# jianwen-xie/Latent-Space-Normalizing-Flow

Hardware: AMD Instinct MI355X
Metric: latent-samples/sec through flow+logdet, nz=128 B=65536 (higher is better)
Workload: dtype bf16x3; 1 GPU; CIFAR-10 flow prior nz=128 f_width=64 f_depth=5 affine, forward+logdet+log-prob, B=65536 synthetic z per evaluation (BASELINE.json configs[2]); rows_per_gpu=65536, global_rows=65536, parallelism=single GPU, streams=3, clock_ramp_launches_before_warmup=600

## Files before the change

### latent-space-normalizing-flow_amd/csrc/lsnf_device.h

```cpp
#pragma once
#include <hip/hip_runtime.h>
#include <type_traits>
#include "lsnf_layout.h"

typedef float f32x16 __attribute__((ext_vector_type(16)));
typedef float f32x4 __attribute__((ext_vector_type(4)));

#define LSNF_WG_THREADS 256
#define LSNF_WG_WAVES 4
#define LSNF_WG_SAMPLES (LSNF_WG_WAVES * 32)

#define LSNF_AS1 __attribute__((address_space(1)))
#define LSNF_AS3 __attribute__((address_space(3)))

static inline hipError_t lsnf_allow_big_lds(const void* kernel, unsigned long long* done_mask) {
    int dev = 0;
    hipError_t e = hipGetDevice(&dev);
    if (e != hipSuccess) return e;
    if (dev >= 0 && dev < 64 && ((*done_mask >> dev) & 1ull)) return hipSuccess;
    e = hipFuncSetAttribute(kernel, hipFuncAttributeMaxDynamicSharedMemorySize, 160 * 1024);
    if (e != hipSuccess) return e;
    if (dev >= 0 && dev < 64) *done_mask |= 1ull << dev;
    return hipSuccess;
}
// ... 7 lines not shown

static inline unsigned long long* lsnf_stamps_buffer() {
#ifdef LSNF_STAMPS
    extern unsigned long long* g_lsnf_stamps;
    if (!g_lsnf_stamps && hipMalloc(&g_lsnf_stamps, sizeof(unsigned long long) * 64 * 4 * 4096) != hipSuccess) g_lsnf_stamps = nullptr;
    return g_lsnf_stamps;
#else
    return nullptr;
#endif
}

template <int HT_, int WT_>
struct LsnfStackCfg {
    static constexpr int HT = HT_, WT = WT_, NZT = 2 * HT_;
    static constexpr int P1 = NZT, P2 = WT, P3 = WT, P4 = 2 * HT, NP = P1 + P2 + P3 + P4;
    static constexpr int KT1 = NZT, KT2 = HT, KT3 = WT, KT4 = WT;
    static constexpr int OFF_S2 = LSNF_FRAG_FLOATS * P1 * KT1;
    static constexpr int OFF_S3 = OFF_S2 + LSNF_FRAG_FLOATS * P2 * KT2;
    static constexpr int OFF_S4 = OFF_S3 + LSNF_FRAG_FLOATS * P3 * KT3;
    static constexpr int FWD_BLOCK = OFF_S4 + LSNF_FRAG_FLOATS * P4 * KT4;
    static constexpr int FWD_CONST = 32 * NP + 32;
    static constexpr int INV_BLOCK = LSNF_FRAG_FLOATS * NZT * NZT;
    static constexpr int INV_CONST = 32 * NZT;
    static constexpr int OFF_B4 = 0;
    static constexpr int OFF_B3 = OFF_B4 + LSNF_FRAG_FLOATS * WT * 2 * HT;
    static constexpr int OFF_B2 = OFF_B3 + LSNF_FRAG_FLOATS * WT * WT;
    static constexpr int OFF_B1 = OFF_B2 + LSNF_FRAG_FLOATS * HT * WT;
    static constexpr int BWD_BLOCK = OFF_B1 + LSNF_FRAG_FLOATS * NZT * NZT;
    static constexpr int MAXKT = (NZT > WT ? NZT : WT);
    static constexpr int SLOT = 2 * MAXKT * LSNF_FRAG_FLOATS;
};

#define LSNF_STATS_SLOTS 64
__device__ __forceinline__ void lsnf_publish_stats(double* stats, double sum_ll, double sum_logdet, int rows, int lane) {
    const unsigned grid = gridDim.x, wg = blockIdx.x;
    unsigned long long* ticket = reinterpret_cast<unsigned long long*>(&stats[2]);
    int last = 0;
    if (lane == 0) {
        const unsigned s = wg % LSNF_STATS_SLOTS;
        double* sub = stats + 8 + 4 * s;
        const double r0 = atomicAdd(&sub[0], sum_ll);
        const double r1 = atomicAdd(&sub[1], sum_logdet);
        unsigned long long inc = 1ull;
        asm volatile("" : "+v"(inc) : "v"(r0), "v"(r1));
        bool slot_done = true;
        if (grid > LSNF_STATS_SLOTS) {
            const unsigned long long n_s = (grid - s + LSNF_STATS_SLOTS - 1) / LSNF_STATS_SLOTS;
            unsigned long long* st = reinterpret_cast<unsigned long long*>(&sub[2]);
            slot_done = atomicAdd(st, inc) == n_s - 1;
            if (slot_done) atomicExch(st, 0ull);
            inc = 1ull;
        }
        if (slot_done) {
            const unsigned long long slots = grid > LSNF_STATS_SLOTS ? LSNF_STATS_SLOTS : grid;
            if (atomicAdd(ticket, inc) == slots - 1) { last = 1; atomicExch(ticket, 0ull); }
        }
    }
    if (__builtin_amdgcn_readfirstlane(last)) {
        unsigned long long* sub = reinterpret_cast<unsigned long long*>(stats + 8 + 4 * lane);
        double fl = __longlong_as_double((long long)atomicExch(&sub[0], 0ull));
        double fd = __longlong_as_double((long long)atomicExch(&sub[1], 0ull));
#pragma unroll
        for (int o = 32; o > 0; o >>= 1) { fl += __shfl_xor(fl, o, 64); fd += __shfl_xor(fd, o, 64); }
        if (lane == 0) { stats[4] = fl; stats[5] = fd; stats[6] = (double)rows; }
    }
}

__device__ __forceinline__ constexpr int lsnf_feat(int r, int h) { return (r & 3) + 8 * (r >> 2) + 4 * h; }

template <int KT, int NW = LSNF_WG_WAVES>
__device__ __forceinline__ void lsnf_issue_panel(const float* __restrict__ gsrc, float* lbuf, int wave, int lane) {
#ifdef LSNF_ABLATE_DMA
    return;
#endif
    constexpr int PIECES = 4 * KT;
    constexpr int PER_WAVE = (PIECES + NW - 1) / NW;
#pragma unroll
    for (int s = 0; s < PER_WAVE; ++s) {
        const int seg = s * NW + wave;
        if (PIECES % NW == 0 || seg < PIECES) {
            const float* g = gsrc + seg * 256 + lane * 4;
            float* l = lbuf + seg * 256;
            __builtin_amdgcn_global_load_lds((const LSNF_AS1 void*)g, (LSNF_AS3 void*)l, 16, 0, 0);
        }
    }
}

__device__ __forceinline__ void lsnf_panel_barrier() {
    asm volatile("s_waitcnt vmcnt(0)" ::: "memory");
#ifndef LSNF_ABLATE_BARRIER
    __syncthreads();
#endif
}

template <int KT>
__device__ __forceinline__ void lsnf_panel_mma(f32x16& acc, const f32x16* in, const float* lbuf, int lane) {
    const f32x4* wp = reinterpret_cast<const f32x4*>(lbuf) + lane;
    __builtin_amdgcn_sched_barrier(0);
// ... 53 lines not shown

__device__ __forceinline__ void lsnf_sigmoid_logsig(float p, float& sig, float& lsig) {
#ifdef LSNF_ABLATE_EPILOGUE
    sig = p * 0.25f + 0.5f; lsig = p; return;
#endif
#ifdef LSNF_OCML_MATH
    const float a = fabsf(p);
    const float e = expf(-a);
    const float r = 1.0f / (1.0f + e);
    const float l = log1pf(e);
    sig = (p >= 0.0f) ? r : e * r;
    lsig = fminf(p, 0.0f) - l;
#else
    float l2;
    lsnf_sigmoid_log2(p, sig, l2);
    lsig = -0.6931471805599453f * l2;
#endif
}

__device__ __forceinline__ float lsnf_pair_add16(float v) {
    const unsigned u = __builtin_bit_cast(unsigned, v);
    const auto r = __builtin_amdgcn_permlane16_swap(u, u, false, false);
    return __builtin_bit_cast(float, (unsigned)r[0]) + __builtin_bit_cast(float, (unsigned)r[1]);
}
__device__ __forceinline__ float lsnf_pair_add32(float v) {
    const unsigned u = __builtin_bit_cast(unsigned, v);
    const auto r = __builtin_amdgcn_permlane32_swap(u, u, false, false);
    return __builtin_bit_cast(float, (unsigned)r[0]) + __builtin_bit_cast(float, (unsigned)r[1]);
}
__device__ __forceinline__ unsigned lsnf_pair_or32(unsigned u) {
    const auto r = __builtin_amdgcn_permlane32_swap(u, u, false, false);
    return (unsigned)r[0] | (unsigned)r[1];
}
__device__ __forceinline__ float lsnf_pair_sum(float v) { return lsnf_pair_add32(v); }

typedef float f32x2 __attribute__((ext_vector_type(2)));
template <int HT>
__device__ __forceinline__ f32x16 lsnf_load_tile(int t, const float* __restrict__ zr, int half, int h, int vw) {
    f32x16 x;
    const int hh = t / HT, tt = t % HT;
#pragma unroll
    for (int g = 0; g < 4; ++g) {
        const int f0 = 32 * tt + 8 * g + 4 * h;
        const int col0 = hh * half + f0;
        if (vw == 4) {
            f32x4 v = {0.f, 0.f, 0.f, 0.f};
            if (f0 < half) v = *reinterpret_cast<const f32x4*>(zr + col0);
            x[4 * g + 0] = v[0]; x[4 * g + 1] = v[1]; x[4 * g + 2] = v[2]; x[4 * g + 3] = v[3];
        } else if (vw == 2) {
            f32x2 v0 = {0.f, 0.f}, v1 = {0.f, 0.f};
            if (f0 < half) v0 = *reinterpret_cast<const f32x2*>(zr + col0);
            if (f0 + 2 < half) v1 = *reinterpret_cast<const f32x2*>(zr + col0 + 2);
            x[4 * g + 0] = v0[0]; x[4 * g + 1] = v0[1]; x[4 * g + 2] = v1[0]; x[4 * g + 3] = v1[1];
        } else {
#pragma unroll
            for (int j = 0; j < 4; ++j) x[4 * g + j] = (f0 + j < half) ? zr[col0 + j] : 0.0f;
        }
    }
    return x;
}

template <int HT>
__device__ __forceinline__ void lsnf_store_tile(int t, const f32x16& x, float* __restrict__ zr, int half, int h, int vw) {
    const int hh = t / HT, tt = t % HT;
#pragma unroll
    for (int g = 0; g < 4; ++g) {
// ... 223 lines not shown
```

### latent-space-normalizing-flow_amd/csrc/lsnf_fwd3p.hip

```cpp
#include <stdlib.h>
#include <type_traits>
#include "lsnf_l16.h"

#if LSNF_L16_PARTS != 3
#error "lsnf_fwd3p.hip is the three-term bf16 kernel"
#endif

#ifndef LSNF_FILLMASK
#define LSNF_FILLMASK 0x7f
#endif

namespace {

struct Fwd3pArgs {
    const float* consts; const float* panels3;
    const float* z_in; const float* objective;
    float* z_out; float* logdet_out; float* ll_out;
    int B, nz, half, n_blocks, vec4;
    double* stats;
    float* hdump; int width;
    float* z_saved; float* act_saved;
    unsigned long long* stamps;
};

#ifdef LSNF_STAMPS
#define P_STAMP(i, INSN)                                                                                \
    do { __builtin_amdgcn_sched_barrier(0);                                                             \
         unsigned long long t_; asm volatile(INSN " %0\n\ts_waitcnt lgkmcnt(0)" : "=s"(t_) :: "memory");  \
         __builtin_amdgcn_sched_barrier(0);                                                             \
         if (a.stamps && lane == 0) a.stamps[(((size_t)blockIdx.x * NWAVES + wave) & 2047) * 64 + (i)] = t_; } while (0)
#else
#define P_STAMP(i, INSN) do {} while (0)
#endif

template <int WT_>
struct Fwd3pCfg : LsnfStackCfg<2, WT_> {
    using S = LsnfStackCfg<2, WT_>;
    static constexpr int F = LSNF_FRAG3_FLOATS;
    static constexpr int OFF3_S2 = F * S::P1 * S::KT1;
    static constexpr int OFF3_S3 = OFF3_S2 + F * S::P2 * S::KT2;
    static constexpr int OFF3_S4 = OFF3_S3 + F * S::P3 * S::KT3;
    static constexpr int BLOCK3 = OFF3_S4 + F * S::P4 * S::KT4;
    static constexpr int SLOT3 = 2 * S::MAXKT * F;
    static constexpr int CONST_FLOATS = S::FWD_CONST;
};

__device__ __forceinline__ void keep(unsigned a, unsigned b, unsigned c) { asm volatile("" :: "v"(a), "v"(b), "v"(c)); }
__device__ __forceinline__ void keep(float a, float b, float c, float d, float e) { asm volatile("" :: "v"(a), "v"(b), "v"(c), "v"(d), "v"(e)); }

struct StepDesc { int acc, tile, s, frag; };
template <int KT> constexpr StepDesc mkstep(int acc, int tl, int in_tile, int kt, int s) { return StepDesc{acc, in_tile, s, ((tl * KT + kt) * 2 + s) * 3}; }

struct Tile16 { f32x4v q[4]; };
struct SplitTile16 { unsigned d[2][3][4]; };

// ... 81 lines not shown
    }
}
template <int ST>
__device__ __forceinline__ void sigmoid_q16(Tile16& p, int q, float* lsum ) {
    const int st = unit_st<ST>(q), qr = unit_quad<ST>(q), r0 = 2 * unit_pair0<ST>(q);
#pragma unroll
    for (int r = r0; r < r0 + 2 * ST; ++r) {
        float sig, l2;
        lsnf_sigmoid_log2(p.q[qr][r], sig, l2);
        p.q[qr][r] = sig; lsum[st] += l2;
    }
    keep(p.q[qr][r0], p.q[qr][r0 + 1], p.q[qr][r0 + 2 * ST - 2], p.q[qr][r0 + 2 * ST - 1], lsum[st]);
}
template <int ST>
__device__ __forceinline__ void couple_q16(Tile16& v, const Tile16& t, const Tile16& sig, int q) {
    const int qr = unit_quad<ST>(q), r0 = 2 * unit_pair0<ST>(q);
#pragma unroll
    for (int r = r0; r < r0 + 2 * ST; ++r) v.q[qr][r] = (v.q[qr][r] + t.q[qr][r]) * sig.q[qr][r];
}

#ifndef LSNF_STASH_AUX
#define LSNF_STASH_AUX 0
#endif
#ifndef LSNF_STASH_PARTS
#define LSNF_STASH_PARTS 7
#endif
typedef unsigned u32x4s __attribute__((ext_vector_type(4)));
struct StashLane { unsigned zoff, soff, moff, msh, hoff; };
struct StashRsrc { __amdgpu_buffer_rsrc_t r[2]; };
__device__ __forceinline__ StashRsrc stash_rsrc(const float* p, unsigned bytes, unsigned second_off) {
    char* c = reinterpret_cast<char*>(const_cast<float*>(p));
    return StashRsrc{{__builtin_amdgcn_make_buffer_rsrc(c, 0, (int)bytes, 0x00020000),
                      __builtin_amdgcn_make_buffer_rsrc(c + second_off, 0, (int)(bytes > second_off ? bytes - second_off : 0u), 0x00020000)}};
}
template <int HT>
__device__ __forceinline__ void stash_row_quad(const StashRsrc& rs, const StashLane& sl, int t, int q, const Tile16& x, int nz, int half, int g) {
    if constexpr (!(LSNF_STASH_PARTS & 4)) return;
    const int ft = q >> 1, st = q & 1, hh = t / HT, tt = t % HT;
    unsigned off = sl.zoff;
    if (st) off += (unsigned)(16 * nz * 4);
    off = (32 * tt + 16 * ft + 4 * g < half) ? off : 0x80000000u;
    const u32x4s v = __builtin_bit_cast(u32x4s, x.q[q]);
    __builtin_amdgcn_raw_buffer_store_b128(v, rs.r[hh], off + (unsigned)((32 * tt + 16 * ft) * 4), 0, LSNF_STASH_AUX);
}
__device__ __forceinline__ void stash_sigma_quad(const StashRsrc& rs, const StashLane& sl, int t, int q, const Tile16& sg) {
    if constexpr (!(LSNF_STASH_PARTS & 2)) return;
    const int ft = q >> 1, st = q & 1;
    const u32x4s v = __builtin_bit_cast(u32x4s, sg.q[q]);
    __builtin_amdgcn_raw_buffer_store_b128(v, rs.r[t], sl.soff + (unsigned)((2 * ft * 64 + 16 * st) * 16), 0, LSNF_STASH_AUX);
}
__device__ __forceinline__ void mask_q16(const Tile16& h, int q, unsigned (&mk)[2][2]) {
    if constexpr (!(LSNF_STASH_PARTS & 1)) return;
    unsigned m = 0;
#pragma unroll
    for (int r = 3; r >= 0; --r) m = __builtin_amdgcn_alignbit(m, __builtin_bit_cast(unsigned, 0.0f - h.q[q][r]), 31);
    mk[q & 1][q >> 1] = m;
    asm volatile("" :: "v"(m));
}
__device__ __forceinline__ void stash_mask_words(const StashRsrc& rs, const StashLane& sl, int tile, const unsigned (&mk)[2][2]) {
    if constexpr (!(LSNF_STASH_PARTS & 1)) return;
    const unsigned w0 = mk[0][0] | (mk[0][1] << 8), w1 = mk[1][0] | (mk[1][1] << 8);
    unsigned x = ((w0 << 16) | w1) << sl.msh;
    x = lsnf_pair_or32(x);
    __builtin_amdgcn_raw_buffer_store_b32(x >> 16, rs.r[0], sl.moff + (unsigned)(tile * 64 * 4), 0, 0);
    __builtin_amdgcn_raw_buffer_store_b32(x & 0xffffu, rs.r[0], sl.moff + (unsigned)((tile * 64 + 16) * 4), 0, 0);
}
// ... 111 lines not shown
    static constexpr int stores(int i) { return QsS23::stores(i) + (((i >= 4 && i < 12) || i >= 13) ? 1 : 0); }
};
struct QxS4 : QsS4 {
    static constexpr int valu(int i) { return QsS4::valu(i) + (i < 4 ? 2 : 0); }
    static constexpr int stores(int i) { return QsS4::stores(i) + (i < 4 ? 1 : 0); }
};
template <class PH> constexpr int stores_after(int last_dma_step) {
    int n = 0;
    for (int i = last_dma_step + 1; i < PH::N; ++i) n += PH::stores(i);
    return n;
}

template <int WT, int NWAVES, int ST, int STASH = 0>
__global__ __launch_bounds__(64 * NWAVES, 1) void lsnf_fwd3q_kernel(const Fwd3pArgs a) {
    static_assert(!STASH || ST == 2, "the stash tile is a wave's 32 rows");
    using TS1a = std::conditional_t<STASH != 0, QsS1a, QhS1a>;
    using TS1b = std::conditional_t<STASH != 0, QsS1b, QhS1b>;
    using TS23 = std::conditional_t<STASH == 2, QxS23, std::conditional_t<STASH != 0, QsS23, QhS23>>;
    using TS4 = std::conditional_t<STASH == 2, QxS4, std::conditional_t<STASH != 0, QsS4, QhS4>>;
    using C = Fwd3pCfg<WT>;
    static_assert(WT == 2, "lsnf_fwd3q_kernel: f_width <= 64 instantiation");
    constexpr int THREADS = 64 * NWAVES;
    constexpr int HT = 2, NZT = 4, F = C::F;
    constexpr int SLOT = C::SLOT3;
    extern __shared__ __attribute__((aligned(16))) float smem[];
    float* cst = smem;
    float* const buf0 = smem + a.n_blocks * C::CONST_FLOATS;
    const int tid = threadIdx.x;
    const int wave = __builtin_amdgcn_readfirstlane(tid >> 6);
    const int lane = tid & 63;
    const int n = lane & 15, g = lane >> 4;
    P_STAMP(0, "s_memtime");
    P_STAMP(50, "s_memrealtime");
    const int n_phases = 4 * a.n_blocks;
    auto phase_src = [&](int k) -> const float* {
        const float* gb = a.panels3 + (size_t)(k >> 2) * C::BLOCK3;
        const int j = k & 3;
        return gb + (j == 0 ? 0 : (j == 1 ? 2 * 4 * F : (j == 2 ? C::OFF3_S2 : C::OFF3_S4)));
    };
    auto sync_issue = [&](int k, auto left) {
#ifdef LSNF_ABL_SKIPSYNC
        if ((LSNF_ABL_SKIPSYNC >> (k & 3)) & 1) return;
#endif
        asm volatile("s_waitcnt vmcnt(%0)" :: "n"(decltype(left)::value) : "memory");
        __syncthreads();
#ifdef LSNF_FWD3Q_BURST_DMA
        if (k + 1 < n_phases) issue_kib<48, NWAVES>(phase_src(k + 1), buf0 + ((k + 1) & 1) * SLOT, wave, lane);
#endif
    };
    constexpr int PER_WAVE = 48 / NWAVES, EVERY = STASH ? 1 : 16 / PER_WAVE, LAST_DMA = (PER_WAVE - 1) * EVERY;
    using Left0 = std::integral_constant<int, 0>;
    using LeftS1a = std::integral_constant<int, stores_after<TS1a>(LAST_DMA)>;
    using LeftS1b = std::integral_constant<int, stores_after<TS1b>(LAST_DMA)>;
    using LeftS23 = std::integral_constant<int, stores_after<TS23>(LAST_DMA) + (STASH == 2 ? 1 : 0)>;
    using LeftS4 = std::integral_constant<int, stores_after<TS4>(LAST_DMA)>;
    const float* dma_src = nullptr; float* dma_dst = nullptr;
    auto dma_arm = [&](int k) {
        dma_src = phase_src(k + 1 < n_phases ? k + 1 : k);
        dma_dst = buf0 + ((k + 1) & 1) * SLOT;
    };
    auto dma_step = [&](auto ic) {
#ifndef LSNF_FWD3Q_BURST_DMA
        constexpr int i = decltype(ic)::value;
        if constexpr (i % EVERY == 0 && i / EVERY < PER_WAVE) issue_piece<NWAVES>(dma_src, dma_dst, i / EVERY, wave, lane);
#endif
    };

    const int wbase = (blockIdx.x * NWAVES + wave) * (16 * ST);
    int sample[2] = {0, 0}, rows[2] = {0, 0}; bool live[2] = {false, false};
#pragma unroll
    for (int st = 0; st < ST; ++st) { sample[st] = wbase + 16 * st + n; live[st] = sample[st] < a.B; rows[st] = live[st] ? sample[st] : a.B - 1; }

    Tile16 v[NZT];
    SplitTile16 xs[NZT];
    Tile16 p1, t1;
    float lsum[2] = {0.0f, 0.0f};
    {
        const Tile16 x0 = load_tile16<HT, ST>(0, a.z_in, rows, a.nz, a.half, g, a.vec4);
        const Tile16 x1 = load_tile16<HT, ST>(1, a.z_in, rows, a.nz, a.half, g, a.vec4);
        v[2] = load_tile16<HT, ST>(2, a.z_in, rows, a.nz, a.half, g, a.vec4);
        v[3] = load_tile16<HT, ST>(3, a.z_in, rows, a.nz, a.half, g, a.vec4);
        __builtin_amdgcn_sched_barrier(0);
        issue_kib<48, NWAVES>(phase_src(0), buf0, wave, lane);
        for (int i = tid; i < a.n_blocks * C::CONST_FLOATS; i += THREADS) cst[i] = a.consts[i];
#pragma unroll
        for (int q = 0; q < 4; ++q) { split_q16<false, ST>(x0, q, xs[0]); split_q16<false, ST>(x1, q, xs[1]); }
        split_q16<false, ST>(v[2], 0, xs[2]); split_q16<false, ST>(v[2], 1, xs[2]);
#pragma unroll
        for (int q = 0; q < 4; ++q)
#pragma unroll
            for (int r = 0; r < 4; ++r) { p1.q[q][r] = 80.0f; t1.q[q][r] = 0.0f; }
    }
    float ell[2];
#pragma unroll
    for (int st = 0; st < 2; ++st) ell[st] = (st < ST && a.objective) ? a.objective[rows[st]] : 0.0f;
    float ss01[2] = {0.0f, 0.0f};
    StashLane sl0 = {0u, 0u, 0u, 0u};
    const LsnfActLayout al = lsnf_act_layout(a.B, HT, WT);
    const unsigned zbytes = (unsigned)a.B * (unsigned)a.nz * 4u, abytes = (unsigned)(al.per_block * 4);
    if constexpr (STASH) {
        const unsigned tile_byte = (unsigned)(wbase >> 5) * (unsigned)(al.per_tile * 4), L = (unsigned)(n + 32 * (g & 1));
        sl0.zoff = ((unsigned)(wbase + n) * (unsigned)a.nz + 4u * g) * 4u;
        sl0.soff = tile_byte + ((unsigned)(g >> 1) * 64u + L) * 16u;
        sl0.moff = tile_byte + (unsigned)(al.mask_off * 4) + L * 4u;
        sl0.msh = 4u * (g >> 1);
        sl0.hoff = (unsigned)(wbase >> 5) * (unsigned)(32 * a.width * 4) + (unsigned)(n * 4 + g) * 16u;
    }
    const LsnfDumpLayout dl = lsnf_dump_layout(a.B, a.nz, a.width);
    const unsigned hbytes = (unsigned)(((size_t)a.B + 31) / 32 * 32 * a.width * 4);
    sync_issue(0, Left0{});
    P_STAMP(1, "s_memtime");

    for (int blk = 0; blk < a.n_blocks; ++blk) {
        const float* cb = cst + blk * C::CONST_FLOATS;
        const bool more = blk + 1 < a.n_blocks;
        const int k0 = 4 * blk;
        SplitTile16 vh[4];
        SplitTile16 h2s[WT];
        Tile16 hh[4], tp[4];
        const bool zs = STASH && a.z_saved != nullptr, as = STASH && a.act_saved != nullptr;
        const float* zc = more ? (zs ? a.z_saved + (size_t)blk * a.B * a.nz : a.z_out) : a.z_out;
        const float* zp = blk > 0 ? (zs ? a.z_saved + (size_t)(blk - 1) * a.B * a.nz : a.z_out) : a.z_out;
        const StashRsrc rs_zc = stash_rsrc(zc, (more && !zs) ? 0u : zbytes, (unsigned)a.half * 4u);
        const StashRsrc rs_zp = stash_rsrc(zp, (blk > 0 && !zs) ? 0u : zbytes, (unsigned)a.half * 4u);
        const StashRsrc rs_ac = stash_rsrc(as ? a.act_saved + (size_t)blk * al.per_block : a.z_out, as ? abytes : 0u, 4096u);
        const StashRsrc rs_ap = stash_rsrc(as ? a.act_saved + (size_t)(blk > 0 ? blk - 1 : 0) * al.per_block : a.z_out, as ? abytes : 0u, 4096u);
        StashLane sl = sl0;
        if constexpr (STASH) asm volatile("" : "+v"(sl.zoff), "+v"(sl.soff), "+v"(sl.moff));
        if constexpr (STASH == 2) asm volatile("" : "+v"(sl.hoff));
        const float* hd = (STASH == 2) ? a.hdump + (size_t)blk * dl.per_block : a.z_out;
        const StashRsrc rs_h1 = stash_rsrc(STASH == 2 ? hd + dl.off_h1 : hd, STASH == 2 ? hbytes : 0u, 4096u);
        const StashRsrc rs_h2 = stash_rsrc(STASH == 2 ? hd + dl.off_h2 : hd, STASH == 2 ? hbytes : 0u, 4096u);
        unsigned mk1[2][2], mk2[2][2], mk3[2][2];

        if (blk == 1) P_STAMP(10, "s_memtime");
        {
            const float* bv = bias_lane_ptr(cb, g);
            if (k0 > 0) sync_issue(k0, LeftS4{});
            dma_arm(k0);
            run_phase16<TS1a, ST>(v, bv, xs, buf0 + (k0 & 1) * SLOT, lane, [&](auto ic) {
                constexpr int i = decltype(ic)::value;
                if constexpr (STASH && i >= 8 && i < 12) stash_row_quad<HT>(rs_zp, sl, 2, i - 8, v[2], a.nz, a.half, g);
                if constexpr (i < 2) split_q16<false, ST>(v[2], 2 + i, xs[2]);
                else if constexpr (i < 6) {
                    sigmoid_q16<ST>(p1, i - 2, lsum);
                    if constexpr (STASH) stash_sigma_quad(rs_ap, sl, 1, i - 2, p1);
                } else if constexpr (i < 8) {
                    couple_q16<ST>(v[3], t1, p1, 2 * (i - 6)); couple_q16<ST>(v[3], t1, p1, 2 * (i - 6) + 1);
                    if constexpr (STASH) { stash_row_quad<HT>(rs_zp, sl, 3, 2 * (i - 6), v[3], a.nz, a.half, g); stash_row_quad<HT>(rs_zp, sl, 3, 2 * (i - 6) + 1, v[3], a.nz, a.half, g); }
                } else if constexpr (i < 12) split_q16<false, ST>(v[3], i - 8, xs[3]);
            }, dma_step);
        }
        if (blk == 1) P_STAMP(11, "s_memtime");
        {
            const float* bv = bias_lane_ptr(cb, g);
            sync_issue(k0 + 1, LeftS1a{});
            dma_arm(k0 + 1);
            run_phase16<TS1b, ST>(v + 2, bv, xs, buf0 + ((k0 + 1) & 1) * SLOT, lane, [&](auto ic) {
                constexpr int i = decltype(ic)::value;
                if constexpr (STASH && i >= 6 && i < 14) stash_row_quad<HT>(rs_zc, sl, (i - 6) >> 2, (i - 6) & 3, v[(i - 6) >> 2], a.nz, a.half, g);
                if constexpr (i >= 8) split_q16<false, ST>(v[(i - 8) >> 2], i & 3, vh[(i - 8) >> 2]);
            }, dma_step);
        }
        if (blk == 1) P_STAMP(12, "s_memtime");
        if (!more) {
            int ln = lane;
            asm volatile("" : "+v"(ln));
            const int smp[2] = {wbase + (ln & 15), wbase + 16 + (ln & 15)};
#pragma unroll
            for (int t = 0; t < HT; ++t) {
                if constexpr (!STASH) store_tile16<HT, ST>(t, v[t], a.z_out, smp, live, a.nz, a.half, g, a.vec4);
#pragma unroll
                for (int ft = 0; ft < 2; ++ft)
#pragma unroll
                    for (int st = 0; st < ST; ++st)
#pragma unroll
                        for (int r = 0; r < 4; ++r) ss01[st] += v[t].q[2 * ft + st][r] * v[t].q[2 * ft + st][r];
            }
        }
#pragma unroll
        for (int st = 0; st < 2; ++st) { ell[st] = ell[st] + cb[32 * C::NP + 0]; ell[st] = ell[st] + cb[32 * C::NP + 1]; }
        {
            static_assert(C::P1 == 4 && C::P2 == 2 && C::P3 == 2, "bias tile indices of the phase tables");
            const float* bv = bias_lane_ptr(cb, g);
            sync_issue(k0 + 2, LeftS1b{});
            dma_arm(k0 + 2);
            run_phase16<TS23, ST>(hh, bv, vh, buf0 + ((k0 + 2) & 1) * SLOT, lane, [&](auto ic) {
                constexpr int i = decltype(ic)::value;
                if constexpr (i >= 4 && i < 8) split_q16<true, ST>(hh[0], i - 4, vh[2]);
                if constexpr (i >= 8 && i < 12) split_q16<true, ST>(hh[1], i - 8, vh[3]);
                if constexpr (i >= 13) split_q16<true, ST>(hh[2], i - 13, h2s[0]);
                if constexpr (STASH) {
                    if constexpr (i >= 4 && i < 8) mask_q16(hh[0], i - 4, mk3);
                    if constexpr (i == 8) stash_mask_words(rs_ac, sl, 0, mk3);
                    if constexpr (i >= 8 && i < 12) mask_q16(hh[1], i - 8, mk1);
                    if constexpr (i >= 13) mask_q16(hh[2], i - 13, mk2);
                }
                if constexpr (STASH == 2) {
                    if constexpr (i >= 4 && i < 8) stash_h_quad(rs_h1, sl, 0, i - 4, hh[0], a.width);
                    if constexpr (i >= 8 && i < 12) stash_h_quad(rs_h1, sl, 1, i - 8, hh[1], a.width);
                    if constexpr (i >= 13) stash_h_quad(rs_h2, sl, 0, i - 13, hh[2], a.width);
                }
            }, dma_step);
        }
// ... 10 lines not shown
            dma_arm(k0 + 3);
            run_phase16<TS4, ST>(tp, bv, h2s, buf0 + ((k0 + 3) & 1) * SLOT, lane, [&](auto ic) {
                constexpr int i = decltype(ic)::value;
                if constexpr (i < 4) split_q16<true, ST>(hh[3], i, h2s[1]);
                if constexpr (STASH) {
                    if constexpr (i < 4) mask_q16(hh[3], i, mk3);
                    if constexpr (i == 6) stash_mask_words(rs_ac, sl, 1, mk1);
                    if constexpr (i == 7) stash_mask_words(rs_ac, sl, WT + 0, mk2);
                    if constexpr (i == 8) stash_mask_words(rs_ac, sl, WT + 1, mk3);
                }
                if constexpr (STASH == 2 && i < 4) stash_h_quad(rs_h2, sl, 1, i, hh[3], a.width);
                if constexpr (i >= 9 && i < 13) { sigmoid_q16<ST>(tp[0], i - 9, lsum); if constexpr (STASH) stash_sigma_quad(rs_ac, sl, 0, i - 9, tp[0]); }
                if constexpr (i == 12) couple_q16<ST>(v[2], tp[1], tp[0], 0);
                if constexpr (i == 13) { couple_q16<ST>(v[2], tp[1], tp[0], 1); couple_q16<ST>(v[2], tp[1], tp[0], 2); couple_q16<ST>(v[2], tp[1], tp[0], 3); }
                if constexpr (i >= 14) split_q16<false, ST>(v[2], i - 14, xs[2]);
            }, dma_step);
            p1 = tp[2]; t1 = tp[3];
        }
        if (blk == 1) P_STAMP(14, "s_memtime");
    }
    P_STAMP(40, "s_memtime");
#pragma unroll
    for (int q = 0; q < 4; ++q) { sigmoid_q16<ST>(p1, q, lsum); couple_q16<ST>(v[3], t1, p1, q); }
    if constexpr (STASH) {
        const bool as = a.act_saved != nullptr;
        const StashRsrc rs_al = stash_rsrc(as ? a.act_saved + (size_t)(a.n_blocks - 1) * al.per_block : a.z_out, as ? abytes : 0u, 4096u);
#pragma unroll
        for (int q = 0; q < 4; ++q) stash_sigma_quad(rs_al, sl0, 1, q, p1);
    }
#pragma unroll
    for (int st = 0; st < ST; ++st) ell[st] = ell[st] + -0.6931471805599453f * l16_group_sum(lsum[st]);

    float ss[2] = {ss01[0], ss01[1]};
    int ln_e = lane;
    asm volatile("" : "+v"(ln_e));
    const int smp_e[2] = {wbase + (ln_e & 15), wbase + 16 + (ln_e & 15)};
#pragma unroll
    for (int t = HT; t < NZT; ++t) {
#pragma unroll
        for (int ft = 0; ft < 2; ++ft)
#pragma unroll
            for (int st = 0; st < ST; ++st)
#pragma unroll
                for (int r = 0; r < 4; ++r) ss[st] += v[t].q[2 * ft + st][r] * v[t].q[2 * ft + st][r];
        store_tile16<HT, ST>(t, v[t], a.z_out, smp_e, live, a.nz, a.half, g, a.vec4);
    }
    float ll[2] = {0.0f, 0.0f};
#pragma unroll
    for (int st = 0; st < ST; ++st) {
        ll[st] = (-0.5f * l16_group_sum(ss[st]) + 1.8378770664093453f) + ell[st];
        if (live[st] && g == 0) {
            const int smp = smp_e[st];
            a.logdet_out[smp] = ell[st];
            if (a.ll_out) a.ll_out[smp] = ll[st];
        }
    }
    asm volatile("s_waitcnt vmcnt(0)" ::: "memory");
    if (a.stats) {
        double dl = 0.0, dd = 0.0;
#pragma unroll
        for (int st = 0; st < ST; ++st)
            if (live[st] && g == 0) { dl += (double)ll[st]; dd += (double)ell[st]; }
#pragma unroll
        for (int o = 8; o > 0; o >>= 1) { dl += __shfl_xor(dl, o, 64); dd += __shfl_xor(dd, o, 64); }
        __syncthreads();
        double* red = reinterpret_cast<double*>(buf0);
        if (lane == 0) { red[2 * wave] = dl; red[2 * wave + 1] = dd; }
        __syncthreads();
        if (wave == 0) {
            double tl = 0.0, td = 0.0;
            for (int w = 0; w < NWAVES; ++w) { tl += red[2 * w]; td += red[2 * w + 1]; }
            lsnf_publish_stats(a.stats, tl, td, a.B, lane);
        }
    }
    P_STAMP(41, "s_memtime");
    P_STAMP(51, "s_memrealtime");
}

size_t fwd3q_lds(int n_blocks) {
    using C = Fwd3pCfg<2>;
    return ((size_t)n_blocks * C::CONST_FLOATS + 2 * (size_t)C::SLOT3) * sizeof(float);
}

template <int WT, int NWAVES, int ST, int STASH = 0>
hipError_t launch_fwd3q_w(const Fwd3pArgs& a, hipStream_t stream) {
    const size_t lds = fwd3q_lds(a.n_blocks);
    auto kern = lsnf_fwd3q_kernel<WT, NWAVES, ST, STASH>;
    static unsigned long long lds_ok = 0;
    if (hipError_t e = lsnf_allow_big_lds((const void*)kern, &lds_ok); e != hipSuccess) return e;
    const unsigned grid = (unsigned)((a.B + 16 * ST * NWAVES - 1) / (16 * ST * NWAVES));
    hipLaunchKernelGGL(kern, dim3(grid), dim3(64 * NWAVES), lds, stream, a);
    return hipGetLastError();
}
}

bool lsnf_forward3q_covers(const LsnfGeo& g, int first_block, int n_blocks, int B, int vec4, const float* z_out,
                           const float* z_saved, const float* act_saved, const float* hdump, int hdump_tiled) {
    if (g.HT != 2 || g.WT != 2 || fwd3q_lds(n_blocks) > 160 * 1024) return false;
    if (hdump && (!hdump_tiled || !act_saved || (n_blocks > 1 && !z_saved) || first_block != 0 || (g.width & 15) ||
                  ((size_t)B + 32) * g.width * 4 >= (1ull << 31))) return false;
    const bool stash = act_saved != nullptr || z_saved != nullptr;
    return !(stash && (vec4 != 4 || (size_t)B * g.nz * 4 >= (1ull << 31) || lsnf_act_layout(B, g.HT, g.WT).per_block * 4 >= (1ull << 31) ||
                       (((size_t)act_saved | (size_t)z_saved | (size_t)z_out) & 15)));
}

hipError_t lsnf_launch_forward3q(const LsnfGeo& g, const float* plan, int first_block, int n_blocks, int B,
                                 const float* z_in, const float* objective, float* z_out, float* logdet_out,
                                 float* ll_out, float* z_saved, float* act_saved, double* stats, int vec4, hipStream_t stream,
                                 float* hdump, int hdump_tiled) {
    if (!lsnf_forward3q_covers(g, first_block, n_blocks, B, vec4, z_out, z_saved, act_saved, hdump, hdump_tiled))
        return hipErrorInvalidValue;
    const bool stash = act_saved != nullptr || z_saved != nullptr;
    Fwd3pArgs a;
    a.consts = plan + g.off_fwd_const + (size_t)first_block * g.fwd_const_floats;
    a.panels3 = plan + g.off_f3b_panels + (size_t)first_block * g.f3_block_floats;
    a.z_in = z_in; a.objective = objective; a.z_out = z_out; a.logdet_out = logdet_out; a.ll_out = ll_out;
    a.B = B; a.nz = g.nz; a.half = g.half; a.n_blocks = n_blocks; a.vec4 = vec4; a.stats = stats;
    a.z_saved = z_saved; a.act_saved = act_saved ? act_saved + (size_t)first_block * lsnf_act_layout(B, g.HT, g.WT).per_block : nullptr;
    a.hdump = hdump; a.width = g.width;
    a.stamps = lsnf_stamps_buffer();
    static const char* shape = getenv("LSNF_FWD3Q_SHAPE");
    const int sh = shape ? atoi(shape) : (B > 128 * 256 ? 82 : (B > 64 * 256 ? 81 : 41));
    if (hdump) return (sh == 82) ? launch_fwd3q_w<2, 8, 2, 2>(a, stream) : launch_fwd3q_w<2, 4, 2, 2>(a, stream);
    if (stash) return (sh == 82) ? launch_fwd3q_w<2, 8, 2, 1>(a, stream) : launch_fwd3q_w<2, 4, 2, 1>(a, stream);
    if (sh == 82) return launch_fwd3q_w<2, 8, 2>(a, stream);
    if (sh == 42) return launch_fwd3q_w<2, 4, 2>(a, stream);
    if (sh == 81) return launch_fwd3q_w<2, 8, 1>(a, stream);
    return launch_fwd3q_w<2, 4, 1>(a, stream);
}
```

### latent-space-normalizing-flow_amd/csrc/lsnf_l16.h

```cpp
#pragma once
#include "lsnf_device.h"

namespace {

typedef __bf16 bf16x2 __attribute__((ext_vector_type(2)));
typedef __bf16 bf16x8 __attribute__((ext_vector_type(8)));
typedef float f32x2v __attribute__((ext_vector_type(2)));
typedef unsigned u32x4 __attribute__((ext_vector_type(4)));

#ifndef LSNF_L16_PARTS
#define LSNF_L16_PARTS 3
#endif
typedef _Float16 f16x2 __attribute__((ext_vector_type(2)));
typedef _Float16 f16x8 __attribute__((ext_vector_type(8)));
#if LSNF_L16_PARTS == 3
typedef bf16x8 l16_op8;
#define LSNF_L16_TERMS(M) M(2, 0) M(0, 2) M(1, 1) M(1, 0) M(0, 1) M(0, 0)
#define LSNF_L16_NTERMS 6
#define LSNF_L16_MFMA __builtin_amdgcn_mfma_f32_16x16x32_bf16
#else
typedef f16x8 l16_op8;
#define LSNF_L16_TERMS(M) M(1, 0) M(0, 1) M(0, 0)
#define LSNF_L16_NTERMS 3
#define LSNF_L16_MFMA __builtin_amdgcn_mfma_f32_16x16x32_f16
#endif
#define L16_FRAG_FLOATS (512 * LSNF_L16_PARTS)

struct Split3 { l16_op8 p[LSNF_L16_PARTS]; };

__device__ __forceinline__ unsigned pk_bf16(float a, float b) {
    const f32x2v v = {a, b};
    return __builtin_bit_cast(unsigned, __builtin_convertvector(v, bf16x2));
}
__device__ __forceinline__ f16x2 pk_f16(float a, float b) {
    const f32x2v v = {a, b};
    return __builtin_convertvector(v, f16x2);
}
template <int KB, int NW>
__device__ __forceinline__ void issue_kib(const float* __restrict__ gsrc, float* lbuf, int wave, int lane) {
    constexpr int PER_WAVE = (KB + NW - 1) / NW;
    const char* base = reinterpret_cast<const char*>(gsrc);
    const unsigned lds0 = (unsigned)(size_t)((LSNF_AS3 char*)lbuf);
    const unsigned lane_off = (unsigned)lane * 16u;
#pragma unroll
    for (int s = 0; s < PER_WAVE; ++s) {
        const int seg = s * NW + wave;
        if (KB % NW == 0 || seg < KB) {
            const char* sb = base + (size_t)seg * 1024u;
            const unsigned m0v = lds0 + (unsigned)seg * 1024u;
            unsigned keep_m0;
            asm volatile("s_mov_b32 %0, m0\n\ts_mov_b32 m0, %3\n\ts_nop 0\n\tglobal_load_lds_dwordx4 %1, %2\n\ts_mov_b32 m0, %0"
                         : "=&s"(keep_m0) : "v"(lane_off), "s"(sb), "s"(m0v) : "memory");
        }
    }
}
template <int NW>
__device__ __forceinline__ void issue_piece(const float* __restrict__ gsrc, float* lbuf, int s, int wave, int lane) {
    const int seg = s * NW + wave;
    const char* sb = reinterpret_cast<const char*>(gsrc) + (size_t)seg * 1024u;
    const unsigned m0v = (unsigned)(size_t)((LSNF_AS3 char*)lbuf) + (unsigned)seg * 1024u;
    const unsigned lane_off = (unsigned)lane * 16u;
    unsigned keep_m0;
    asm volatile("s_mov_b32 %0, m0\n\ts_mov_b32 m0, %3\n\ts_nop 0\n\tglobal_load_lds_dwordx4 %1, %2\n\ts_mov_b32 m0, %0"
                 : "=&s"(keep_m0) : "v"(lane_off), "s"(sb), "s"(m0v) : "memory");
}
template <int NW>
struct Pipe3 {
    float* buf0; int slot, cur, wave, lane;
    template <int KB> __device__ __forceinline__ void prime(const float* src) { issue_kib<KB, NW>(src, buf0, wave, lane); cur = 0; }
    template <int KB_NEXT> __device__ __forceinline__ const float* acquire(const float* next) {
        lsnf_panel_barrier();
        if (next != nullptr) issue_kib<KB_NEXT, NW>(next, buf0 + (cur ^ 1) * slot, wave, lane);
        const float* ready = buf0 + cur * slot;
        cur ^= 1;
        return ready;
    }
};
__device__ __forceinline__ constexpr int first_kib(int NT, int KT) { return 2 * LSNF_L16_PARTS * KT * (NT >= 2 ? 2 : 1); }

#define LSNF_F3_TERMS(M) M(2, 0) M(0, 2) M(1, 1) M(1, 0) M(0, 1) M(0, 0)

typedef float f32x4v __attribute__((ext_vector_type(4)));

__device__ __forceinline__ constexpr int l16_feat0(int ft, int g) { return 16 * ft + 4 * g; }

template <int HT, class R>
__device__ __forceinline__ f32x16 l16_load_tile(int t, const float* __restrict__ z, const R* rows, int nz, int half, int g, int vw) {
    f32x16 x;
    const int hh = t / HT, tt = t % HT;
#pragma unroll
    for (int ft = 0; ft < 2; ++ft)
#pragma unroll
        for (int st = 0; st < 2; ++st) {
            const int f0 = 32 * tt + l16_feat0(ft, g), col0 = hh * half + f0, b = (2 * ft + st) * 4;
            const float* zr = z + (long)rows[st] * (long)nz;
            if (vw == 4) {
                f32x4 v = {0.f, 0.f, 0.f, 0.f};
// ... 224 lines not shown
```

Before: 741.0 million latent-samples/s.

## Overlap final stores with stats atomics and use buffer stores for outputs

The epilogue now issues the stats atomics first and runs the z/logdet/ll stores while those atomics are in flight, removing the vmcnt(0) wait before publishing. When the output fits a 32-bit buffer range, final stores go through raw buffer stores with out-of-range offsets instead of per-lane predicated stores. The cross-lane f64 reduction switches from shuffles to DPP, and the redundant last-phase panel DMA is masked off by setting exec from a scalar flag. Writing exec directly in inline asm and forcing it back to -1 is fragile, because it assumes the wave was fully active at that point.

```diff
diff --git a/latent-space-normalizing-flow_amd/csrc/lsnf_device.h b/latent-space-normalizing-flow_amd/csrc/lsnf_device.h
--- a/latent-space-normalizing-flow_amd/csrc/lsnf_device.h
+++ b/latent-space-normalizing-flow_amd/csrc/lsnf_device.h
@@ -63,15 +63,26 @@
 };
 
 #define LSNF_STATS_SLOTS 64
-__device__ __forceinline__ void lsnf_publish_stats(double* stats, double sum_ll, double sum_logdet, int rows, int lane) {
+template <class Mid>
+__device__ __forceinline__ void lsnf_publish_stats_around(bool active, double* stats, double sum_ll, double sum_logdet, int rows, int lane,
+                                                          Mid&& mid) {
     const unsigned grid = gridDim.x, wg = blockIdx.x;
     unsigned long long* ticket = reinterpret_cast<unsigned long long*>(&stats[2]);
+    const unsigned s = wg % LSNF_STATS_SLOTS;
+    const bool lead = active && lane == 0;
+    double r0, r1;
+    if (lead) {
+        unsigned zero = 0u;
+        asm volatile("" : "+v"(zero));
+        double* sub = stats + 8 + 4 * s + zero;
+        r0 = atomicAdd(&sub[0], sum_ll);
+        r1 = atomicAdd(&sub[1], sum_logdet);
+    }
+    mid();
+    if (!active) return;
     int last = 0;
-    if (lane == 0) {
-        const unsigned s = wg % LSNF_STATS_SLOTS;
+    if (lead) {
         double* sub = stats + 8 + 4 * s;
-        const double r0 = atomicAdd(&sub[0], sum_ll);
-        const double r1 = atomicAdd(&sub[1], sum_logdet);
         unsigned long long inc = 1ull;
         asm volatile("" : "+v"(inc) : "v"(r0), "v"(r1));
         bool slot_done = true;
@@ -95,6 +106,9 @@
         for (int o = 32; o > 0; o >>= 1) { fl += __shfl_xor(fl, o, 64); fd += __shfl_xor(fd, o, 64); }
         if (lane == 0) { stats[4] = fl; stats[5] = fd; stats[6] = (double)rows; }
     }
+}
+__device__ __forceinline__ void lsnf_publish_stats(double* stats, double sum_ll, double sum_logdet, int rows, int lane) {
+    lsnf_publish_stats_around(true, stats, sum_ll, sum_logdet, rows, lane, [] {});
 }
 
 __device__ __forceinline__ constexpr int lsnf_feat(int r, int h) { return (r & 3) + 8 * (r >> 2) + 4 * h; }
@@ -214,6 +228,21 @@
     const auto r = __builtin_amdgcn_permlane32_swap(u, u, false, false);
     return (unsigned)r[0] | (unsigned)r[1];
 }
+template <int CTRL>
+__device__ __forceinline__ double lsnf_dpp_f64(double v) {
+    const unsigned long long u = __builtin_bit_cast(unsigned long long, v);
+    const int lo = (int)(unsigned)u, hi = (int)(unsigned)(u >> 32);
+    const unsigned plo = (unsigned)__builtin_amdgcn_update_dpp(lo, lo, CTRL, 0xf, 0xf, false);
+    const unsigned phi = (unsigned)__builtin_amdgcn_update_dpp(hi, hi, CTRL, 0xf, 0xf, false);
+    return __builtin_bit_cast(double, ((unsigned long long)phi << 32) | plo);
+}
+__device__ __forceinline__ double lsnf_row16_sum_f64(double v) {
+    v += lsnf_dpp_f64<0xB1>(v);
+    v += lsnf_dpp_f64<0x4E>(v);
+    v += lsnf_dpp_f64<0x141>(v);
+    v += lsnf_dpp_f64<0x140>(v);
+    return v;
+}
 __device__ __forceinline__ float lsnf_pair_sum(float v) { return lsnf_pair_add32(v); }
 
 typedef float f32x2 __attribute__((ext_vector_type(2)));
diff --git a/latent-space-normalizing-flow_amd/csrc/lsnf_fwd3p.hip b/latent-space-normalizing-flow_amd/csrc/lsnf_fwd3p.hip
--- a/latent-space-normalizing-flow_amd/csrc/lsnf_fwd3p.hip
+++ b/latent-space-normalizing-flow_amd/csrc/lsnf_fwd3p.hip
@@ -21,6 +21,7 @@
     float* hdump; int width;
     float* z_saved; float* act_saved;
     unsigned long long* stamps;
+    int raw_out;
 };
 
 #ifdef LSNF_STAMPS
@@ -168,6 +169,12 @@
     char* c = reinterpret_cast<char*>(const_cast<float*>(p));
     return StashRsrc{{__builtin_amdgcn_make_buffer_rsrc(c, 0, (int)bytes, 0x00020000),
                       __builtin_amdgcn_make_buffer_rsrc(c + second_off, 0, (int)(bytes > second_off ? bytes - second_off : 0u), 0x00020000)}};
+}
+__device__ __forceinline__ StashRsrc final_rsrc(const float* p, unsigned bytes, unsigned second_off) {
+    char* c = reinterpret_cast<char*>(const_cast<float*>(p));
+    const int second = __builtin_amdgcn_readfirstlane((int)(bytes > second_off ? bytes - second_off : 0u));
+    return StashRsrc{{__builtin_amdgcn_make_buffer_rsrc(c, 0, (int)bytes, 0x00020000),
+                      __builtin_amdgcn_make_buffer_rsrc(c + second_off, 0, second, 0x00020000)}};
 }
 template <int HT>
 __device__ __forceinline__ void stash_row_quad(const StashRsrc& rs, const StashLane& sl, int t, int q, const Tile16& x, int nz, int half, int g) {
@@ -345,6 +352,7 @@
     const int n = lane & 15, g = lane >> 4;
     P_STAMP(0, "s_memtime");
     P_STAMP(50, "s_memrealtime");
+    __builtin_assume(a.n_blocks >= 1);
     const int n_phases = 4 * a.n_blocks;
     auto phase_src = [&](int k) -> const float* {
         const float* gb = a.panels3 + (size_t)(k >> 2) * C::BLOCK3;
@@ -367,15 +375,17 @@
     using LeftS1b = std::integral_constant<int, stores_after<TS1b>(LAST_DMA)>;
     using LeftS23 = std::integral_constant<int, stores_after<TS23>(LAST_DMA) + (STASH == 2 ? 1 : 0)>;
     using LeftS4 = std::integral_constant<int, stores_after<TS4>(LAST_DMA)>;
-    const float* dma_src = nullptr; float* dma_dst = nullptr;
+    const float* dma_src = nullptr; float* dma_dst = nullptr; unsigned dma_on = 0u;
     auto dma_arm = [&](int k) {
-        dma_src = phase_src(k + 1 < n_phases ? k + 1 : k);
+        const bool next = k + 1 < n_phases;
+        dma_src = phase_src(next ? k + 1 : k);
         dma_dst = buf0 + ((k + 1) & 1) * SLOT;
+        dma_on = (unsigned)__builtin_amdgcn_readfirstlane(next ? -1 : 0);
     };
     auto dma_step = [&](auto ic) {
 #ifndef LSNF_FWD3Q_BURST_DMA
         constexpr int i = decltype(ic)::value;
-        if constexpr (i % EVERY == 0 && i / EVERY < PER_WAVE) issue_piece<NWAVES>(dma_src, dma_dst, i / EVERY, wave, lane);
+        if constexpr (i % EVERY == 0 && i / EVERY < PER_WAVE) issue_piece<NWAVES>(dma_src, dma_dst, i / EVERY, wave, lane, dma_on);
 #endif
     };
 
@@ -419,6 +429,23 @@
         sl0.msh = 4u * (g >> 1);
         sl0.hoff = (unsigned)(wbase >> 5) * (unsigned)(32 * a.width * 4) + (unsigned)(n * 4 + g) * 16u;
     }
+    auto final_lane = [&](int& ln) {
+        ln = lane;
+        asm volatile("" : "+v"(ln));
+        StashLane s = {0u, 0u, 0u, 0u, 0u};
+        s.zoff = ((unsigned)(wbase + (ln & 15)) * (unsigned)a.nz + 4u * (unsigned)(ln >> 4)) * 4u;
+        return s;
+    };
+    auto store_final_tile = [&](const StashRsrc& rs, const StashLane& s, int gq, auto tc, const Tile16& x) {
+        constexpr int t = decltype(tc)::value;
+#pragma unroll
+        for (int ft = 0; ft < 2; ++ft)
+#pragma unroll
+            for (int st = 0; st < ST; ++st) {
+                stash_row_quad<HT>(rs, s, t, 2 * ft + st, x, a.nz, a.half, gq);
+                __builtin_amdgcn_sched_barrier(0);
+            }
+    };
     const LsnfDumpLayout dl = lsnf_dump_layout(a.B, a.nz, a.width);
     const unsigned hbytes = (unsigned)(((size_t)a.B + 31) / 32 * 32 * a.width * 4);
     sync_issue(0, Left0{});
@@ -477,12 +504,24 @@
         }
         if (blk == 1) P_STAMP(12, "s_memtime");
         if (!more) {
-            int ln = lane;
-            asm volatile("" : "+v"(ln));
-            const int smp[2] = {wbase + (ln & 15), wbase + 16 + (ln & 15)};
+            if constexpr (!STASH) {
+                if (a.raw_out) {
+                    int ln;
+                    const StashLane slf = final_lane(ln);
+                    const StashRsrc rs_f = final_rsrc(a.z_out, zbytes, (unsigned)a.half * 4u);
+                    store_final_tile(rs_f, slf, ln >> 4, std::integral_constant<int, 0>{}, v[0]);
+                    store_final_tile(rs_f, slf, ln >> 4, std::integral_constant<int, 1>{}, v[1]);
+                } else {
+                    int ln = lane;
+                    asm volatile("" : "+v"(ln));
+                    const int smp[2] = {wbase + (ln & 15), wbase + 16 + (ln & 15)};
+                    const bool lv[2] = {smp[0] < a.B, smp[1] < a.B};
+#pragma unroll
+                    for (int t = 0; t < HT; ++t) store_tile16<HT, ST>(t, v[t], a.z_out, smp, lv, a.nz, a.half, ln >> 4, a.vec4);
+                }
+            }
 #pragma unroll
             for (int t = 0; t < HT; ++t) {
-                if constexpr (!STASH) store_tile16<HT, ST>(t, v[t], a.z_out, smp, live, a.nz, a.half, g, a.vec4);
 #pragma unroll
                 for (int ft = 0; ft < 2; ++ft)
 #pragma unroll
@@ -559,46 +598,63 @@
     for (int st = 0; st < ST; ++st) ell[st] = ell[st] + -0.6931471805599453f * l16_group_sum(lsum[st]);
 
     float ss[2] = {ss01[0], ss01[1]};
-    int ln_e = lane;
-    asm volatile("" : "+v"(ln_e));
+#pragma unroll
+    for (int t = HT; t < NZT; ++t)
+#pragma unroll
+        for (int ft = 0; ft < 2; ++ft)
+#pragma unroll
+            for (int st = 0; st < ST; ++st)
+#pragma unroll
+                for (int r = 0; r < 4; ++r) ss[st] += v[t].q[2 * ft + st][r] * v[t].q[2 * ft + st][r];
+    float ll[2] = {0.0f, 0.0f};
+#pragma unroll
+    for (int st = 0; st < ST; ++st) ll[st] = (-0.5f * l16_group_sum(ss[st]) + 1.8378770664093453f) + ell[st];
+    int ln_e;
+    const StashLane sl_e = final_lane(ln_e);
+    const int g_e = ln_e >> 4;
     const int smp_e[2] = {wbase + (ln_e & 15), wbase + 16 + (ln_e & 15)};
-#pragma unroll
-    for (int t = HT; t < NZT; ++t) {
-#pragma unroll
-        for (int ft = 0; ft < 2; ++ft)
-#pragma unroll
-            for (int st = 0; st < ST; ++st)
-#pragma unroll
-                for (int r = 0; r < 4; ++r) ss[st] += v[t].q[2 * ft + st][r] * v[t].q[2 * ft + st][r];
-        store_tile16<HT, ST>(t, v[t], a.z_out, smp_e, live, a.nz, a.half, g, a.vec4);
-    }
-    float ll[2] = {0.0f, 0.0f};
-#pragma unroll
-    for (int st = 0; st < ST; ++st) {
-        ll[st] = (-0.5f * l16_group_sum(ss[st]) + 1.8378770664093453f) + ell[st];
-        if (live[st] && g == 0) {
-            const int smp = smp_e[st];
-            a.logdet_out[smp] = ell[st];
-            if (a.ll_out) a.ll_out[smp] = ll[st];
-        }
-    }
-    asm volatile("s_waitcnt vmcnt(0)" ::: "memory");
+    const bool publish = a.stats != nullptr && wave == 0;
+    double tl = 0.0, td = 0.0;
     if (a.stats) {
         double dl = 0.0, dd = 0.0;
 #pragma unroll
         for (int st = 0; st < ST; ++st)
-            if (live[st] && g == 0) { dl += (double)ll[st]; dd += (double)ell[st]; }
-#pragma unroll
-        for (int o = 8; o > 0; o >>= 1) { dl += __shfl_xor(dl, o, 64); dd += __shfl_xor(dd, o, 64); }
-        __syncthreads();
+            if (smp_e[st] < a.B && g_e == 0) { dl += (double)ll[st]; dd += (double)ell[st]; }
+        dl = lsnf_row16_sum_f64(dl); dd = lsnf_row16_sum_f64(dd);
         double* red = reinterpret_cast<double*>(buf0);
         if (lane == 0) { red[2 * wave] = dl; red[2 * wave + 1] = dd; }
         __syncthreads();
-        if (wave == 0) {
-            double tl = 0.0, td = 0.0;
+        if (publish)
             for (int w = 0; w < NWAVES; ++w) { tl += red[2 * w]; td += red[2 * w + 1]; }
-            lsnf_publish_stats(a.stats, tl, td, a.B, lane);
-        }
+    }
+    if (a.raw_out) {
+      lsnf_publish_stats_around(publish, a.stats, tl, td, a.B, lane, [&] {
+        const StashRsrc rs_f = final_rsrc(a.z_out, zbytes, (unsigned)a.half * 4u);
+        store_final_tile(rs_f, sl_e, g_e, std::integral_constant<int, 2>{}, v[2]);
+        store_final_tile(rs_f, sl_e, g_e, std::integral_constant<int, 3>{}, v[3]);
+        const unsigned rbytes = (unsigned)a.B * 4u;
+        const __amdgpu_buffer_rsrc_t rs_ld = __builtin_amdgcn_make_buffer_rsrc(reinterpret_cast<char*>(a.logdet_out), 0, (int)rbytes, 0x00020000);
+        const __amdgpu_buffer_rsrc_t rs_ll = __builtin_amdgcn_make_buffer_rsrc(reinterpret_cast<char*>(a.ll_out ? a.ll_out : a.logdet_out), 0,
+                                                                                 (int)(a.ll_out ? rbytes : 0u), 0x00020000);
+        const unsigned roff = g_e == 0 ? (unsigned)smp_e[0] * 4u : 0x80000000u;
+#pragma unroll
+        for (int st = 0; st < ST; ++st) {
+            __builtin_amdgcn_raw_buffer_store_b32(__builtin_bit_cast(unsigned, ell[st]), rs_ld, roff + (unsigned)(64 * st), 0, 0);
+            __builtin_amdgcn_raw_buffer_store_b32(__builtin_bit_cast(unsigned, ll[st]), rs_ll, roff + (unsigned)(64 * st), 0, 0);
+        }
+      });
+    } else {
+      lsnf_publish_stats_around(publish, a.stats, tl, td, a.B, lane, [&] {
+        const bool live_e[2] = {smp_e[0] < a.B, smp_e[1] < a.B};
+#pragma unroll
+        for (int t = HT; t < NZT; ++t) store_tile16<HT, ST>(t, v[t], a.z_out, smp_e, live_e, a.nz, a.half, g_e, a.vec4);
+#pragma unroll
+        for (int st = 0; st < ST; ++st)
+            if (live_e[st] && g_e == 0) {
+                a.logdet_out[smp_e[st]] = ell[st];
+                if (a.ll_out) a.ll_out[smp_e[st]] = ll[st];
+            }
+      });
     }
     P_STAMP(41, "s_memtime");
     P_STAMP(51, "s_memrealtime");
@@ -646,6 +702,7 @@
     a.z_saved = z_saved; a.act_saved = act_saved ? act_saved + (size_t)first_block * lsnf_act_layout(B, g.HT, g.WT).per_block : nullptr;
     a.hdump = hdump; a.width = g.width;
     a.stamps = lsnf_stamps_buffer();
+    a.raw_out = vec4 == 4 && ((size_t)B + 256) * g.nz * 4 < (1ull << 31);
     static const char* shape = getenv("LSNF_FWD3Q_SHAPE");
     const int sh = shape ? atoi(shape) : (B > 128 * 256 ? 82 : (B > 64 * 256 ? 81 : 41));
     if (hdump) return (sh == 82) ? launch_fwd3q_w<2, 8, 2, 2>(a, stream) : launch_fwd3q_w<2, 4, 2, 2>(a, stream);
diff --git a/latent-space-normalizing-flow_amd/csrc/lsnf_l16.h b/latent-space-normalizing-flow_amd/csrc/lsnf_l16.h
--- a/latent-space-normalizing-flow_amd/csrc/lsnf_l16.h
+++ b/latent-space-normalizing-flow_amd/csrc/lsnf_l16.h
@@ -55,14 +55,15 @@
     }
 }
 template <int NW>
-__device__ __forceinline__ void issue_piece(const float* __restrict__ gsrc, float* lbuf, int s, int wave, int lane) {
+__device__ __forceinline__ void issue_piece(const float* __restrict__ gsrc, float* lbuf, int s, int wave, int lane, unsigned on) {
     const int seg = s * NW + wave;
     const char* sb = reinterpret_cast<const char*>(gsrc) + (size_t)seg * 1024u;
     const unsigned m0v = (unsigned)(size_t)((LSNF_AS3 char*)lbuf) + (unsigned)seg * 1024u;
     const unsigned lane_off = (unsigned)lane * 16u;
     unsigned keep_m0;
-    asm volatile("s_mov_b32 %0, m0\n\ts_mov_b32 m0, %3\n\ts_nop 0\n\tglobal_load_lds_dwordx4 %1, %2\n\ts_mov_b32 m0, %0"
-                 : "=&s"(keep_m0) : "v"(lane_off), "s"(sb), "s"(m0v) : "memory");
+    asm volatile("s_mov_b32 %0, m0\n\ts_mov_b32 m0, %3\n\ts_mov_b32 exec_lo, %4\n\ts_mov_b32 exec_hi, %4\n\tglobal_load_lds_dwordx4 %1, %2\n\t"
+                 "s_mov_b64 exec, -1\n\ts_mov_b32 m0, %0"
+                 : "=&s"(keep_m0) : "v"(lane_off), "s"(sb), "s"(m0v), "s"(on) : "memory");
 }
 template <int NW>
 struct Pipe3 {
```

New measurement: 730.4 million latent-samples/s. -1.4%, worse.
